# kenoogl/CubeZ

Measured on AMD Instinct MI355X. Metric: MLUPS (lattice updates/s), 512^3 FP32 Jacobi per GPU, higher is better.
Workload: dtype f32

## Files before the change

### cubez_amd/csrc/cz_k_jac3.h

```cpp

template <class T>
__device__ __forceinline__ T* uniform_global(T* p) {
  auto g = (__attribute__((address_space(1))) T*)p;
  asm("" : "+s"(g));
  return (T*)g;
}

__device__ __forceinline__ unsigned lane_offset(unsigned o) {
  asm("" : "+v"(o));
  return o;
}

template <int V>
__device__ __forceinline__ void complete_here(Vec<V>& x) {
  static_assert(V == 2 || V == 4, "one constraint per component");
  if constexpr (V == 4) asm volatile("" : "+v"(x.v[0]), "+v"(x.v[1]), "+v"(x.v[2]), "+v"(x.v[3]));
  else asm volatile("" : "+v"(x.v[0]), "+v"(x.v[1]));
}

template <int V, int TB, int UNIT, int MED, int GATE = 0>
__global__ void __launch_bounds__(TB, 1)
jac3_k(const REAL* __restrict__ U, const REAL* __restrict__ B, REAL* __restrict__ W, Coef c, Geom2 g, double* partials,
       const int* __restrict__ skip, Fin2 fin) {
  if (skip != nullptr && *skip != 0) return;
  extern __shared__ __attribute__((aligned(16))) char smem[];
  const int t = threadIdx.x;
  const int R = g.R;
  constexpr int LV = TB;
  const DeepLds<V> lds = deep_lds<V, LV, 3>(smem, R);
  const int LU = lds.LU;
  Vec<V>* ldsU = lds.U;
  Vec<V>* ldsF = lds.F;
  double* wsum = lds.wsum;

  const PassItem it = pass_item<V>(g);
  const int ja = it.ja, jb = it.jb;

  double acc1 = 0.0, acc2 = 0.0, acc3 = 0.0;
  const typename std::conditional<GATE != 0, GatedDiv<MED>, typename std::conditional<MED != 0, MediumDiv, HoistedDiv>::type>::type dv{fastdiv_init(c.dd)};

  if (it.work) {
    const long long e2_0 = it.fb - 2 * (long long)R;
    const size_t PB = (size_t)g.PSB;
    const RowView<V> rv = row_view<V>(g, it);
    const int x = t;
    const long long f = e2_0 + x;
    unsigned bo = rv.off_of(f);
    const VecMask mk = vec_mask<V>(g, it, f);
    const unsigned inbox = mk.rows ? mk.bits : 0u;
    const unsigned own = (x >= 2 * R && x < LV - 2 * R && mk.rows && mk.kown) ? mk.bits : 0u;
    const bool wave2 = __builtin_amdgcn_ballot_w64(x >= R && x < LV - R) != 0ull;
    const bool wave3 = __builtin_amdgcn_ballot_w64(own != 0) != 0ull;
    OuterRow h = outer_row<V, TB>(rv, LV, it.fb - 3 * (long long)R, f);
    const bool waveh = __builtin_amdgcn_ballot_w64(h.has) != 0ull;
    const char* Ub = reinterpret_cast<const char*>(U);
    const char* Bb = reinterpret_cast<const char*>(B);
    char* Wb = reinterpret_cast<char*>(W);

    const int q0 = ja - 2;
    Vec<V> uA, uB, bA, bB, hx = zerov<V>();
    {
      const Vec<V> t2 = ld16<V>(Ub + (size_t)rv.pl(q0 - 1) * PB, rv.lim(bo, rv.pl(q0 - 1)));
      const Vec<V> t1 = ld16<V>(Ub + (size_t)rv.pl(q0) * PB, rv.lim(bo, rv.pl(q0)));
      Vec<V> h1 = zerov<V>();
      if (waveh) {
        h1 = ld16<V>(Ub + (size_t)rv.pl(q0) * PB, rv.lim(h.bo, rv.pl(q0)));
        hx = ld16<V>(Ub + (size_t)rv.pl(q0 + 1) * PB, rv.lim(h.bo, rv.pl(q0 + 1)));
      }
      uA = ld16<V>(Ub + (size_t)rv.pl(q0 + 1) * PB, rv.lim(bo, rv.pl(q0 + 1)));
      bA = ld16<V>(Bb + (size_t)rv.pl(q0) * PB, rv.lim(bo, rv.pl(q0)));
      ldsU[(size_t)((q0 - 1) & 1) * LU + R + x] = t2;
      ldsU[(size_t)(q0 & 1) * LU + R + x] = t1;
      if (h.has) ldsU[(size_t)(q0 & 1) * LU + h.hl] = h1;
    }
    Vec<V> bq1 = zerov<V>(), bq2 = zerov<V>();
    __syncthreads();

    const int x_first = __builtin_amdgcn_readfirstlane(x), x_last = __builtin_amdgcn_readlane(x, 63);
    auto stage = [&](const Vec<V>* cur, const Vec<V>* prv, const Vec<V>& nxt, const Vec<V>& bb, unsigned msk, unsigned cnt,
                     double& acc) __attribute__((always_inline)) -> Vec<V> {
      const Vec<V> pc = lds_ld<V>(cur + x);
      const Vec<V> im = lds_ld<V>(cur + x - R);
      const Vec<V> ip = lds_ld<V>(cur + x + R);
      const Vec<V> pm = lds_ld<V>(prv + x);
      const REAL elo = reinterpret_cast<const REAL*>(cur)[(long long)x_first * V - 1];
      const REAL ehi = reinterpret_cast<const REAL*>(cur)[(long long)(x_last + 1) * V];
      const REAL kl = lane_shr1(elo, pc.v[V - 1]);
      const REAL kr = lane_shl1(ehi, pc.v[0]);
      return relax_vec<V, UNIT>(pc, im, ip, pm, nxt, kl, kr, bb, c, dv, msk, cnt, acc);
    };

    const char* uN = Ub;
    const char* bN = Bb;
    char* wN = Wb;
    auto step = [&](auto inner, const int q, Vec<V>& uc, Vec<V>& un, Vec<V>& b1, Vec<V>& bn, Vec<V>& b2, Vec<V>& b3) __attribute__((always_inline)) {
      constexpr bool INNER = decltype(inner)::value;
      const char *up, *bp;
      unsigned uo, bo1, ho;
      if constexpr (INNER) {
        uN = uniform_global(uN), bN = uniform_global(bN), wN = uniform_global(wN);
        bo = lane_offset(bo), h.bo = lane_offset(h.bo);
        up = uN, bp = bN, uo = bo, bo1 = bo, ho = h.bo;
      } else {
        const int qu = rv.pl(q + 2 <= jb + 3 ? q + 2 : jb + 3), qb = rv.pl(q + 1 <= jb + 2 ? q + 1 : jb + 2);
        up = Ub + (size_t)qu * PB, bp = Bb + (size_t)qb * PB;
        uo = rv.lim(bo, qu), bo1 = rv.lim(bo, qb), ho = rv.lim(h.bo, qu);
      }
      un = ld16<V>(up, uo);
      bn = ld16<V>(bp, bo1);
      const int p1 = q, p2 = q - 1, p3 = q - 2;
      auto upd = [&](int p) -> unsigned { return (INNER || (p >= g.jj0 && p <= g.jj1)) ? inbox : 0u; };
      auto cnt = [&](int p) -> unsigned { return (INNER || (p >= ja && p <= jb)) ? own : 0u; };
      const Vec<V>* cU = ldsU + (size_t)(p1 & 1) * LU + R;
      const Vec<V>* pU = ldsU + (size_t)((p1 - 1) & 1) * LU + R;
      Vec<V>* F1 = ldsF;
      Vec<V>* F2 = ldsF + (size_t)2 * LV;
      Vec<V> v1 = stage(cU, pU, uc, b1, upd(p1), cnt(p1), acc1);
      complete_here<V>(v1);
      if (waveh) {
        if (h.has) ldsU[(size_t)((p1 + 1) & 1) * LU + h.hl] = hx;
        hx = ld16<V>(up, ho);
      }
      Vec<V> v2 = v1;
      if (wave2) v2 = stage(F1 + (size_t)(p2 & 1) * LV, F1 + (size_t)((p2 - 1) & 1) * LV, v1, b2, upd(p2), cnt(p2), acc2);
      if ((INNER || p3 >= ja) && wave3) {
        const Vec<V> o = stage(F2 + (size_t)(p3 & 1) * LV, F2 + (size_t)((p3 - 1) & 1) * LV, v2, b3, own, own, acc3);
        store_owned<V>(INNER ? wN : Wb + (size_t)p3 * PB, bo, own, o);
      }
      F1[(size_t)(p1 & 1) * LV + x] = v1;
      F2[(size_t)(p2 & 1) * LV + x] = v2;
      Vec<V>* nU = ldsU + (size_t)((p1 + 1) & 1) * LU;
      nU[R + x] = uc;
      if constexpr (!INNER) b3 = b2, b2 = b1;
      if constexpr (INNER) uN += PB, bN += PB, wN += PB;
      __syncthreads();
    };
    const int qi = jb < g.jlast - 3 ? jb : g.jlast - 3;
    int q = q0;
#pragma nounroll
    for (int phase = 0; phase < 2; phase++) {
      const int qg = phase == 0 ? ja + 1 : jb + 2;
      for (;;) {
        step(std::false_type{}, q, uA, uB, bA, bB, bq1, bq2);
        if (++q > qg) break;
        step(std::false_type{}, q, uB, uA, bB, bA, bq1, bq2);
        if (++q > qg) break;
      }
      if (phase == 0) {
        uN = Ub + (size_t)(q + 2) * PB, bN = Bb + (size_t)(q + 1) * PB, wN = Wb + (size_t)(q - 2) * PB;
        for (; q + 3 <= qi; q += 4) {
          step(std::true_type{}, q, uA, uB, bA, bB, bq1, bq2);
          step(std::true_type{}, q + 1, uB, uA, bB, bq2, bA, bq1);
          step(std::true_type{}, q + 2, uA, uB, bq2, bq1, bB, bA);
          step(std::true_type{}, q + 3, uB, uA, bq1, bA, bq2, bB);
        }
      }
    }
  }

  const double acc[3] = {acc1, acc2, acc3};
  pass_epilogue<TB, 3>(acc, partials, fin, wsum);
}
```

### cubez_amd/csrc/cz_k_pass.h

```cpp
struct Geom2 {
  int R;
  long long PSV;
  int nkp = 0;
  long long PSB = 0;
  int jlast = 0;
  unsigned last_off = 0;
  int nwin = 1;
  int hv = 0;
  int KT = 1 << 30;
  int KW = 0;
  int nsegw = 0;
  int kk0, kk1, jj0, jj1;
  long long F0, Fend;
  int kk0a, kk1a, jj0a, jj1a;
  long long F0a, Fenda;
  int nseg, TJ, S;
  int par;
  int zero_u;
  int band;
  const int* map;
};

struct BSrc {
  const REAL* x = nullptr;
  const REAL* y = nullptr;
  const REAL* z = nullptr;
  REAL* out = nullptr;
  REAL a = 0, b = 0;
  const REAL* pa = nullptr;
};

struct Fin2 {
  double* dst = nullptr;
  int do_check = 0, itr = 0;
  int single = 0;
  const double* extra = nullptr;
  int n_extra = 0;
  double res_normal = 0.0, eps = 0.0;
  double* hist = nullptr;
  int* flag = nullptr;
  int* conv_itr = nullptr;
  unsigned* counter = nullptr;
};

template <int V>
__device__ __forceinline__ unsigned colour_bits(int base) {
  const unsigned even = (V == 4) ? 0x5u : (V == 2) ? 0x1u : 0x1u;
  const unsigned odd = (V == 4) ? 0xAu : (V == 2) ? 0x2u : 0x0u;
  return (base & 1) ? odd : even;
}

struct PlainDiv {
  REAL d;
  __device__ __forceinline__ REAL operator()(REAL n) const { return n / d; }
};
struct HoistedDiv {
  FastDiv<REAL> f;
  __device__ __forceinline__ REAL operator()(REAL n) const { return fastdiv(n, f); }
};

struct ShortDiv {
  FastDiv<REAL> f;
  __device__ __forceinline__ REAL operator()(REAL n) const { return shortdiv(n, f); }
};

struct MediumDiv {
  FastDiv<REAL> f;
  __device__ __forceinline__ REAL operator()(REAL n) const { return mediumdiv(n, f); }
};

__device__ __forceinline__ float uniform_real(float x) { return __builtin_bit_cast(float, __builtin_amdgcn_readfirstlane(__builtin_bit_cast(int, x))); }
__device__ __forceinline__ double uniform_real(double x) {
  const unsigned long long b = __builtin_bit_cast(unsigned long long, x);
  const unsigned lo = __builtin_amdgcn_readfirstlane((unsigned)b), hi = __builtin_amdgcn_readfirstlane((unsigned)(b >> 32));
  return __builtin_bit_cast(double, ((unsigned long long)hi << 32) | lo);
}
template <int MED>
struct GatedDiv {
  FastDiv<REAL> f;
  REAL T;
  __device__ __forceinline__ explicit GatedDiv(const FastDiv<REAL>& f_) : f(f_), T(uniform_real(f_.T)) {}
  template <int V>
  __device__ __forceinline__ void vec(const REAL (&n)[V], REAL (&q)[V]) const {
    if (__builtin_expect(gated_none_huge<V>(n, T), 1)) {
#pragma unroll
      for (int cc = 0; cc < V; cc++) q[cc] = gated_tail<MED>(n[cc], f);
    } else {
#pragma unroll
      for (int cc = 0; cc < V; cc++) q[cc] = general_tail<MED>(n[cc], f);
    }
  }
};
template <class DIV>
struct has_vec_entry : std::false_type {};
template <int MED>
struct has_vec_entry<GatedDiv<MED>> : std::true_type {};

template <int V, int UNIT = 0, class DIV>
__device__ __forceinline__ Vec<V> relax_vec(const Vec<V>& pc, const Vec<V>& im, const Vec<V>& ip, const Vec<V>& pm,
                                            const Vec<V>& pn, REAL kl, REAL kr, const Vec<V>& bb, const Coef& c, const DIV& dv,
                                            unsigned mask, unsigned count_mask, double& acc) {
  Vec<V> o;
#if defined(CZ_P2_RES_GROUP)
  REAL grp = (REAL)0;
#endif
  constexpr bool BY_VECTOR = has_vec_entry<DIV>::value;
  REAL nv[V], qv[V];
  if constexpr (BY_VECTOR) {
#pragma unroll
    for (int cc = 0; cc < V; cc++) {
      const REAL km1 = (cc == 0) ? kl : pc.v[cc > 0 ? cc - 1 : 0];
      const REAL kp1 = (cc == V - 1) ? kr : pc.v[cc < V - 1 ? cc + 1 : V - 1];
      nv[cc] = offdiag_sum<UNIT>(c, ip.v[cc], im.v[cc], pn.v[cc], pm.v[cc], kp1, km1) - bb.v[cc];
    }
    dv.template vec<V>(nv, qv);
  }
#pragma unroll
  for (int cc = 0; cc < V; cc++) {
    const REAL pp = pc.v[cc];
    REAL qd;
    if constexpr (BY_VECTOR) {
      qd = qv[cc];
    } else {
      const REAL km1 = (cc == 0) ? kl : pc.v[cc > 0 ? cc - 1 : 0];
      const REAL kp1 = (cc == V - 1) ? kr : pc.v[cc < V - 1 ? cc + 1 : V - 1];
      const REAL ss = offdiag_sum<UNIT>(c, ip.v[cc], im.v[cc], pn.v[cc], pm.v[cc], kp1, km1);
      qd = dv(ss - bb.v[cc]);
    }
    const REAL dp = (qd - pp) * c.omg;
    const REAL d2 = dp * dp;
    o.v[cc] = (mask & (1u << cc)) ? pp + dp : pp;
#if defined(CZ_P2_NO_RES)
    (void)d2, (void)count_mask, (void)acc;
#elif defined(CZ_P2_RES_GROUP)
    grp += (count_mask & (1u << cc)) ? d2 : (REAL)0;
#else
    acc += (double)((count_mask & (1u << cc)) ? d2 : (REAL)0);
#endif
  }
#if defined(CZ_P2_RES_GROUP)
  acc += (double)grp;
#endif
  return o;
}

template <int V>
__device__ __forceinline__ Vec<V> relax_vec_maf(const Vec<V>& pc, const Vec<V>& im, const Vec<V>& ip, const Vec<V>& pm, const Vec<V>& pn,
                                                REAL kl, REAL kr, const Vec<V>& bb, REAL XG, REAL XGG, REAL YE, REAL YEE, const Vec<V>& ZT,
                                                const Vec<V>& ZTT, REAL omg, unsigned mask, unsigned count_mask, double& acc) {
  Vec<V> o;
#pragma unroll
  for (int cc = 0; cc < V; cc++) {
    const REAL pp = pc.v[cc];
    const REAL km1 = (cc == 0) ? kl : pc.v[cc > 0 ? cc - 1 : 0];
    const REAL kp1 = (cc == V - 1) ? kr : pc.v[cc < V - 1 ? cc + 1 : V - 1];
    const MafW w = maf_weights(XG, XGG, YE, YEE, ZT.v[cc], ZTT.v[cc]);
    const REAL rp = w.w1 * ip.v[cc] + w.w2 * im.v[cc] + w.w3 * pn.v[cc] + w.w4 * pm.v[cc] + w.w5 * kp1 + w.w6 * km1 + bb.v[cc];
    const REAL dp = (rp / w.dd - pp) * omg;
    const REAL d2 = dp * dp;
    o.v[cc] = (mask & (1u << cc)) ? pp + dp : pp;
    acc += (double)((count_mask & (1u << cc)) ? d2 : (REAL)0);
  }
  return o;
}

template <int V>
__device__ __forceinline__ Vec<V> ld16(const char* plane, unsigned byte_off) {
  typedef typename NatVec<V>::type nv;
  typedef nv unv __attribute__((aligned(sizeof(REAL))));
  const nv x = *reinterpret_cast<const unv*>(plane + byte_off);
  Vec<V> r;
  __builtin_memcpy(&r, &x, sizeof(r));
  return r;
}
template <int V>
__device__ __forceinline__ void st16(char* plane, unsigned byte_off, const Vec<V>& x) {
  typedef typename NatVec<V>::type nv;
  typedef nv unv __attribute__((aligned(sizeof(REAL))));
  nv y;
  __builtin_memcpy(&y, &x, sizeof(y));
  *reinterpret_cast<unv*>(plane + byte_off) = y;
}

template <int V>
__device__ __forceinline__ Vec<V> lds_ld(const Vec<V>* p) {
  typedef typename NatVec<V>::type nv;
  nv x = *reinterpret_cast<const nv*>(p);
  asm("" : "+v"(x));
  Vec<V> r;
  __builtin_memcpy(&r, &x, sizeof(r));
  return r;
}

struct PassItem {
  int win, seg, chunk;
  int kw0;
  long long fb;
  int ja, jb;
  bool work;
};
template <int V>
__device__ __forceinline__ PassItem pass_item(const Geom2& g) {
  PassItem it;
  const int lb = blockIdx.x;
  int seg, chunk;
  if (g.map != nullptr) {
    seg = g.map[2 * lb];
    chunk = g.map[2 * lb + 1];
  } else {
    const int x = lb & 7, r = lb >> 3;
    const int base = g.nseg >> 3, rem = g.nseg & 7, bmax = base + (rem ? 1 : 0);
    const int blen = base + (x < rem ? 1 : 0);
    const int sl = r % bmax;
    chunk = r / bmax;
    seg = (sl < blen) ? x * base + min(x, rem) + sl : g.nseg;
  }
  int win = 0;
  if (g.nwin > 1 && seg < g.nseg) {
    win = seg / g.nsegw;
    seg -= win * g.nsegw;
  } else if (g.nwin > 1) {
    seg = g.nsegw;
  }
  const int nseg_w = (g.nwin > 1) ? g.nsegw : g.nseg;
  it.win = win, it.seg = seg, it.chunk = chunk;
  it.kw0 = win * g.KW - g.hv * V;
  it.fb = (seg < nseg_w) ? g.F0 + (long long)seg * g.S : g.Fend;
  it.ja = g.jj0 + chunk * g.TJ;
  it.jb = it.ja + g.TJ - 1;
  if (it.jb > g.jj1) it.jb = g.jj1;
  it.work = it.ja <= it.jb && it.fb < g.Fend;
  return it;
}

template <int V>
struct RowView {
  int R, nkp, kw0, jlast;
  unsigned last_off;
  long long vlast;
  __device__ __forceinline__ unsigned off_of(long long f) const {
    if (f < 0) f = 0;
    if (f > vlast) f = vlast;
    const long long r = f / R;
    long long el = r * nkp + kw0 + (f - r * R) * V;
    el = el < 0 ? 0 : el;
    return (unsigned)(el * (long long)sizeof(REAL));
  }
  __device__ __forceinline__ unsigned lim(unsigned off, int plane) const { return plane == jlast ? (off < last_off ? off : last_off) : off; }
  __device__ __forceinline__ int pl(int p) const { return p < 0 ? 0 : (p > jlast ? jlast : p); }
};
template <int V>
__device__ __forceinline__ RowView<V> row_view(const Geom2& g, const PassItem& it) {
  return RowView<V>{g.R, g.nkp, it.kw0, g.jlast, g.last_off, g.PSV - 1};
}

struct VecMask {
  unsigned bits, bits1;
  bool rows, rows1;
  bool kown;
  int pbase;
};
template <int V>
__device__ __forceinline__ VecMask vec_mask(const Geom2& g, const PassItem& it, long long f) {
  const long long fc = f < 0 ? 0 : f;
  const long long row = fc / g.R;
  const int kv = (int)(fc - row * g.R);
  const int kb = it.kw0 + kv * V;
  VecMask m;
  m.bits = 0, m.bits1 = 0;
#pragma unroll
  for (int cc = 0; cc < V; cc++) {
    const int kk = kb + cc;
    if (kk >= g.kk0a && kk <= g.kk1a) m.bits1 |= 1u << cc;
    if (kk >= g.kk0 && kk <= g.kk1) m.bits |= 1u << cc;
  }
  m.rows = f >= g.F0 && f < g.Fend;
  m.rows1 = f >= g.F0a && f < g.Fenda;
  m.kown = kv >= g.hv && kv < g.hv + g.KT;
  m.pbase = kb + (int)row + g.par;
  return m;
}

struct OuterRow {
  bool has;
  int hl;
  unsigned bo;
};
template <int V, int TB>
__device__ __forceinline__ OuterRow outer_row(const RowView<V>& rv, int LV, long long f_outer0, long long f_own) {
  const int t = threadIdx.x, R = rv.R;
  OuterRow h;
  h.has = (t < R) || (t >= TB - R);
  h.hl = (t < R) ? t : (LV + R + (t - (TB - R)));
  h.bo = rv.off_of(h.has ? f_outer0 + h.hl : f_own);
  return h;
}

template <int V>
__device__ __forceinline__ void store_owned(char* plane, unsigned bo, unsigned own, const Vec<V>& x) {
  if (own == (1u << V) - 1) {
    st16<V>(plane, bo, x);
  } else if (own != 0) {
    REAL* p = reinterpret_cast<REAL*>(plane + bo);
#pragma unroll
    for (int cc = 0; cc < V; cc++)
      if (own & (1u << cc)) p[cc] = x.v[cc];
  }
}

template <int V>
struct DeepLds {
  int LU;
  Vec<V>* U;
  Vec<V>* F;
  double* wsum;
};
template <int V, int LV, int D>
__device__ __forceinline__ DeepLds<V> deep_lds(char* smem, int R) {
  DeepLds<V> l;
  l.LU = LV + 2 * R;
  l.U = reinterpret_cast<Vec<V>*>(smem) + R;
  l.F = l.U + (size_t)2 * l.LU;
  l.wsum = reinterpret_cast<double*>(l.F + (size_t)(2 * (D - 1)) * LV + R);
  return l;
}

template <int TB, int N>
__device__ __forceinline__ void pass_finalize(const double* partials, int nblk, const Fin2& fin, double* wsum) {
  const int t = threadIdx.x;
  double x[N];
#pragma unroll
  for (int s = 0; s < N; s++) x[s] = 0.0;
  for (int i = t; i < nblk; i += TB) {
#pragma unroll
    for (int s = 0; s < N; s++) x[s] += __hip_atomic_load(&partials[s * nblk + i], __ATOMIC_RELAXED, __HIP_MEMORY_SCOPE_AGENT);
  }
  for (int i = t; i < fin.n_extra; i += TB) {
#pragma unroll
    for (int s = 0; s < N; s++) x[s] += fin.extra[s * fin.n_extra + i];
  }
  double tot[N];
#pragma unroll
  for (int s = 0; s < N; s++) {
    __syncthreads();
    tot[s] = block_sum<TB>(x[s], wsum);
  }
  if (t == 0) {
    const bool single = N == 2 && fin.single;
    if (single) tot[0] = tot[0] + tot[1];
    const int nit = single ? 1 : N;
    for (int s = 0; s < nit; s++) fin.dst[s] = tot[s];
    if (fin.do_check) {
      for (int s = 0; s < nit; s++) {
        const double r = sqrt(tot[s] * fin.res_normal);
        fin.hist[fin.itr + s] = r;
        if (r < fin.eps) {
          *fin.flag = 1;
          *fin.conv_itr = fin.itr + s;
          break;
        }
      }
    }
    *fin.counter = 0u;
  }
}

template <int TB, int N>
__device__ __forceinline__ void pass_epilogue(const double (&acc)[N], double* partials, const Fin2& fin, double* wsum) {
  const int lb = blockIdx.x, nblk = gridDim.x;
  double s[N];
#pragma unroll
  for (int n = 0; n < N; n++) {
    __syncthreads();
    s[n] = block_sum<TB>(acc[n], wsum);
  }
  int* last_flag = reinterpret_cast<int*>(wsum + 16);
  if (threadIdx.x == 0) {
#pragma unroll
    for (int n = 0; n < N; n++) __hip_atomic_store(&partials[n * nblk + lb], s[n], __ATOMIC_RELAXED, __HIP_MEMORY_SCOPE_AGENT);
    *last_flag = arrive_and_test_last(fin.counter, nblk);
  }
  __syncthreads();
  if (*last_flag) pass_finalize<TB, N>(partials, nblk, fin, wsum);
}
```

### cubez_amd/csrc/cz_k_rb4.h

```cpp
template <int V, int TB, int UNIT>
__global__ void __launch_bounds__(TB, 1)
rb4_k(const REAL* __restrict__ U, const REAL* __restrict__ B, REAL* __restrict__ W, Coef c, Geom2 g, double* partials,
      const int* __restrict__ skip, Fin2 fin) {
  if (skip != nullptr && *skip != 0) return;
  extern __shared__ __attribute__((aligned(16))) char smem[];
  const int t = threadIdx.x;
  const int R = g.R;
  constexpr int LV = TB;
  const DeepLds<V> lds = deep_lds<V, LV, 4>(smem, R);
  const int LU = lds.LU;
  Vec<V>* ldsU = lds.U;
  Vec<V>* ldsF = lds.F;
  double* wsum = lds.wsum;

  const PassItem it = pass_item<V>(g);
  const int ja = it.ja, jb = it.jb;

  double acc1 = 0.0, acc2 = 0.0;
  const HoistedDiv dv{fastdiv_init(c.dd)};

  if (it.work) {
    const long long e3_0 = it.fb - 3 * (long long)R;
    const size_t PB = (size_t)g.PSB;
    const RowView<V> rv = row_view<V>(g, it);
    int x;
    {
      const int off = (int)(((e3_0 % R) + R) % R);
      const int L0 = off == 0 ? R : R - off;
      int nA = L0;
      for (int st = L0 + R; st < LV; st += 2 * R) nA += min(R, LV - st);
      if (t < nA) {
        const int m = t - L0, j = m / R;
        x = t < L0 ? t : L0 + R + 2 * R * j + (m - j * R);
      } else {
        const int n = t - nA, j = n / R;
        x = L0 + 2 * R * j + (n - j * R);
      }
    }
    const long long f = e3_0 + x;
    const unsigned bo = rv.off_of(f);
    const VecMask mk = vec_mask<V>(g, it, f);
    const int pbase = mk.pbase;
    const unsigned inbox = mk.rows ? mk.bits : 0u;
    const unsigned own = (x >= 3 * R && x < LV - 3 * R && mk.rows && mk.kown) ? mk.bits : 0u;
    const OuterRow h = outer_row<V, TB>(rv, LV, it.fb - 4 * (long long)R, f);
    const char* Ub = reinterpret_cast<const char*>(U);
    const char* Bb = reinterpret_cast<const char*>(B);
    char* Wb = reinterpret_cast<char*>(W);

    const int q0 = ja - 3;
    Vec<V> uA, uB, bA, bB, hx;
    {
      const Vec<V> t2 = ld16<V>(Ub + (size_t)rv.pl(q0 - 1) * PB, rv.lim(bo, rv.pl(q0 - 1)));
      const Vec<V> t1 = ld16<V>(Ub + (size_t)rv.pl(q0) * PB, rv.lim(bo, rv.pl(q0)));
      const Vec<V> h1 = ld16<V>(Ub + (size_t)rv.pl(q0) * PB, rv.lim(h.bo, rv.pl(q0)));
      uA = ld16<V>(Ub + (size_t)rv.pl(q0 + 1) * PB, rv.lim(bo, rv.pl(q0 + 1)));
      bA = ld16<V>(Bb + (size_t)rv.pl(q0) * PB, rv.lim(bo, rv.pl(q0)));
      ldsU[(size_t)((q0 - 1) & 1) * LU + R + x] = t2;
      ldsU[(size_t)(q0 & 1) * LU + R + x] = t1;
      if (h.has) ldsU[(size_t)(q0 & 1) * LU + h.hl] = h1;
    }
    Vec<V> bq1 = zerov<V>(), bq2 = zerov<V>(), bq3 = zerov<V>();
    __syncthreads();

    const int x_first = __builtin_amdgcn_readfirstlane(x), x_last = __builtin_amdgcn_readlane(x, 63);
    struct Ops {
      Vec<V> pc, im, ip;
      REAL elo, ehi;
    };
    auto fetch = [&](const Vec<V>* cur) __attribute__((always_inline)) -> Ops {
      Ops o;
      o.pc = lds_ld<V>(cur + x);
      o.im = lds_ld<V>(cur + x - R);
      o.ip = lds_ld<V>(cur + x + R);
      o.elo = reinterpret_cast<const REAL*>(cur)[(long long)x_first * V - 1];
      o.ehi = reinterpret_cast<const REAL*>(cur)[(long long)(x_last + 1) * V];
      return o;
    };
    auto compute = [&](const Ops& o, const Vec<V>* cur, const Vec<V>* prv, const Vec<V>& nxt, const Vec<V>& bb, int p, int colour, unsigned msk, unsigned cnt, double& acc,
                       const bool first = false) __attribute__((always_inline)) -> Vec<V> {
      const Vec<V> pm = lds_ld<V>(prv + x);
      const REAL kl = lane_shr1(o.elo, o.pc.v[V - 1]);
      REAL kr = lane_shl1(o.ehi, o.pc.v[0]);
      if (first) kr = (x == LV - 1) ? reinterpret_cast<const REAL*>(cur)[(long long)LV * V] : kr;
      const bool sc = ((pbase + p + colour) & 1) != 0;
      return relax_vec_rb_branch<V>(o.pc, o.im, o.ip, pm, nxt, kl, kr, bb, sc, msk, cnt, acc,
                             [&](REAL pp, REAL ipv, REAL imv, REAL pnv, REAL pmv, REAL kp1, REAL km1, REAL bv, REAL, REAL) {
                               const REAL ss = offdiag_sum<UNIT>(c, ipv, imv, pnv, pmv, kp1, km1);
                               return (dv(ss - bv) - pp) * c.omg;
                             });
    };

    auto step = [&](const int q, Vec<V>& uc, Vec<V>& un, Vec<V>& b1, Vec<V>& bn) __attribute__((always_inline)) {
      {
        const int qu = rv.pl(q + 2 <= jb + 4 ? q + 2 : jb + 4), qb = rv.pl(q + 1 <= jb + 3 ? q + 1 : jb + 3);
        hx = ld16<V>(Ub + (size_t)rv.pl(q + 1) * PB, rv.lim(h.bo, rv.pl(q + 1)));
        un = ld16<V>(Ub + (size_t)qu * PB, rv.lim(bo, qu));
        bn = ld16<V>(Bb + (size_t)qb * PB, rv.lim(bo, qb));
      }
      const int p1 = q, p2 = q - 1, p3 = q - 2, p4 = q - 3;
      auto upd = [&](int p) -> unsigned { return (p >= g.jj0 && p <= g.jj1) ? inbox : 0u; };
      auto cnt = [&](int p) -> unsigned { return (p >= ja && p <= jb) ? own : 0u; };
      const Vec<V>* cU = ldsU + (size_t)(p1 & 1) * LU + R;
      const Vec<V>* pU = ldsU + (size_t)((p1 - 1) & 1) * LU + R;
      Vec<V>* F1 = ldsF;
      Vec<V>* F2 = ldsF + (size_t)2 * LV;
      Vec<V>* F3 = ldsF + (size_t)4 * LV;
      const Ops o1 = fetch(cU);
      const Ops o2 = fetch(F1 + (size_t)(p2 & 1) * LV);
      const Vec<V> v1 = compute(o1, cU, pU, uc, b1, p1, 0, upd(p1), cnt(p1), acc1, true);
      const Ops o3 = fetch(F2 + (size_t)(p3 & 1) * LV);
      const Vec<V> v2 = compute(o2, nullptr, F1 + (size_t)((p2 - 1) & 1) * LV, v1, bq1, p2, 1, upd(p2), cnt(p2), acc1);
      const Ops o4 = fetch(F3 + (size_t)(p4 & 1) * LV);
      const Vec<V> v3 = compute(o3, nullptr, F2 + (size_t)((p3 - 1) & 1) * LV, v2, bq2, p3, 0, upd(p3), cnt(p3), acc2);
      if (p4 >= ja && __builtin_amdgcn_ballot_w64(own != 0) != 0ull) {
        const Vec<V> o = compute(o4, nullptr, F3 + (size_t)((p4 - 1) & 1) * LV, v3, bq3, p4, 1, own, own, acc2);
        store_owned<V>(Wb + (size_t)p4 * PB, bo, own, o);
      }
      F1[(size_t)(p1 & 1) * LV + x] = v1;
      F2[(size_t)(p2 & 1) * LV + x] = v2;
      F3[(size_t)(p3 & 1) * LV + x] = v3;
      Vec<V>* nU = ldsU + (size_t)((p1 + 1) & 1) * LU;
      nU[R + x] = uc;
      if (h.has) nU[h.hl] = hx;
      bq3 = bq2, bq2 = bq1, bq1 = b1;
      __syncthreads();
    };
    for (int q = q0;; q += 2) {
      step(q, uA, uB, bA, bB);
      if (q + 1 > jb + 3) break;
      step(q + 1, uB, uA, bB, bA);
      if (q + 2 > jb + 3) break;
    }
  }

  const double acc[2] = {acc1, acc2};
  pass_epilogue<TB, 2>(acc, partials, fin, wsum);
}
```

Measured before the change: 1.080 million.

## Port jac3 inner-loop specialization to rb4 kernel with rotating B registers

Moves the uniform_global, lane_offset and complete_here helpers into the shared pass header so the red-black 4-stage kernel can use them. The rb4 step is split into boundary and inner variants: the inner loop walks scalar base pointers with no clamping or range checks and is unrolled by six, rotating the B pipeline registers instead of copying them. Halo loads are skipped for waves with no halo lanes and issued mid-step to overlap with compute, and wave-uniform ballots gate the owned stage. The aim is less address arithmetic, fewer register moves and fewer scalar/vector conversions per plane, at the cost of more code and higher register pressure.

```diff
diff --git a/cubez_amd/csrc/cz_k_jac3.h b/cubez_amd/csrc/cz_k_jac3.h
--- a/cubez_amd/csrc/cz_k_jac3.h
+++ b/cubez_amd/csrc/cz_k_jac3.h
@@ -1,22 +1,4 @@
 
-template <class T>
-__device__ __forceinline__ T* uniform_global(T* p) {
-  auto g = (__attribute__((address_space(1))) T*)p;
-  asm("" : "+s"(g));
-  return (T*)g;
-}
-
-__device__ __forceinline__ unsigned lane_offset(unsigned o) {
-  asm("" : "+v"(o));
-  return o;
-}
-
-template <int V>
-__device__ __forceinline__ void complete_here(Vec<V>& x) {
-  static_assert(V == 2 || V == 4, "one constraint per component");
-  if constexpr (V == 4) asm volatile("" : "+v"(x.v[0]), "+v"(x.v[1]), "+v"(x.v[2]), "+v"(x.v[3]));
-  else asm volatile("" : "+v"(x.v[0]), "+v"(x.v[1]));
-}
 
 template <int V, int TB, int UNIT, int MED, int GATE = 0>
 __global__ void __launch_bounds__(TB, 1)
diff --git a/cubez_amd/csrc/cz_k_pass.h b/cubez_amd/csrc/cz_k_pass.h
--- a/cubez_amd/csrc/cz_k_pass.h
+++ b/cubez_amd/csrc/cz_k_pass.h
@@ -192,6 +192,25 @@
   return r;
 }
 
+template <class T>
+__device__ __forceinline__ T* uniform_global(T* p) {
+  auto g = (__attribute__((address_space(1))) T*)p;
+  asm("" : "+s"(g));
+  return (T*)g;
+}
+
+__device__ __forceinline__ unsigned lane_offset(unsigned o) {
+  asm("" : "+v"(o));
+  return o;
+}
+
+template <int V>
+__device__ __forceinline__ void complete_here(Vec<V>& x) {
+  static_assert(V == 2 || V == 4, "one constraint per component");
+  if constexpr (V == 4) asm volatile("" : "+v"(x.v[0]), "+v"(x.v[1]), "+v"(x.v[2]), "+v"(x.v[3]));
+  else asm volatile("" : "+v"(x.v[0]), "+v"(x.v[1]));
+}
+
 struct PassItem {
   int win, seg, chunk;
   int kw0;
diff --git a/cubez_amd/csrc/cz_k_rb4.h b/cubez_amd/csrc/cz_k_rb4.h
--- a/cubez_amd/csrc/cz_k_rb4.h
+++ b/cubez_amd/csrc/cz_k_rb4.h
@@ -38,22 +38,28 @@
       }
     }
     const long long f = e3_0 + x;
-    const unsigned bo = rv.off_of(f);
+    unsigned bo = rv.off_of(f);
     const VecMask mk = vec_mask<V>(g, it, f);
     const int pbase = mk.pbase;
     const unsigned inbox = mk.rows ? mk.bits : 0u;
     const unsigned own = (x >= 3 * R && x < LV - 3 * R && mk.rows && mk.kown) ? mk.bits : 0u;
-    const OuterRow h = outer_row<V, TB>(rv, LV, it.fb - 4 * (long long)R, f);
+    const bool wave4 = __builtin_amdgcn_ballot_w64(own != 0) != 0ull;
+    OuterRow h = outer_row<V, TB>(rv, LV, it.fb - 4 * (long long)R, f);
+    const bool waveh = __builtin_amdgcn_ballot_w64(h.has) != 0ull;
     const char* Ub = reinterpret_cast<const char*>(U);
     const char* Bb = reinterpret_cast<const char*>(B);
     char* Wb = reinterpret_cast<char*>(W);
 
     const int q0 = ja - 3;
-    Vec<V> uA, uB, bA, bB, hx;
+    Vec<V> uA, uB, bA, bB, hx = zerov<V>();
     {
       const Vec<V> t2 = ld16<V>(Ub + (size_t)rv.pl(q0 - 1) * PB, rv.lim(bo, rv.pl(q0 - 1)));
       const Vec<V> t1 = ld16<V>(Ub + (size_t)rv.pl(q0) * PB, rv.lim(bo, rv.pl(q0)));
-      const Vec<V> h1 = ld16<V>(Ub + (size_t)rv.pl(q0) * PB, rv.lim(h.bo, rv.pl(q0)));
+      Vec<V> h1 = zerov<V>();
+      if (waveh) {
+        h1 = ld16<V>(Ub + (size_t)rv.pl(q0) * PB, rv.lim(h.bo, rv.pl(q0)));
+        hx = ld16<V>(Ub + (size_t)rv.pl(q0 + 1) * PB, rv.lim(h.bo, rv.pl(q0 + 1)));
+      }
       uA = ld16<V>(Ub + (size_t)rv.pl(q0 + 1) * PB, rv.lim(bo, rv.pl(q0 + 1)));
       bA = ld16<V>(Bb + (size_t)rv.pl(q0) * PB, rv.lim(bo, rv.pl(q0)));
       ldsU[(size_t)((q0 - 1) & 1) * LU + R + x] = t2;
@@ -61,6 +67,7 @@
       if (h.has) ldsU[(size_t)(q0 & 1) * LU + h.hl] = h1;
     }
     Vec<V> bq1 = zerov<V>(), bq2 = zerov<V>(), bq3 = zerov<V>();
+    Vec<V> bX = zerov<V>();
     __syncthreads();
 
     const int x_first = __builtin_amdgcn_readfirstlane(x), x_last = __builtin_amdgcn_readlane(x, 63);
@@ -84,23 +91,36 @@
       REAL kr = lane_shl1(o.ehi, o.pc.v[0]);
       if (first) kr = (x == LV - 1) ? reinterpret_cast<const REAL*>(cur)[(long long)LV * V] : kr;
       const bool sc = ((pbase + p + colour) & 1) != 0;
-      return relax_vec_rb_branch<V>(o.pc, o.im, o.ip, pm, nxt, kl, kr, bb, sc, msk, cnt, acc,
+      const Vec<V> r = relax_vec_rb_branch<V>(o.pc, o.im, o.ip, pm, nxt, kl, kr, bb, sc, msk, cnt, acc,
                              [&](REAL pp, REAL ipv, REAL imv, REAL pnv, REAL pmv, REAL kp1, REAL km1, REAL bv, REAL, REAL) {
                                const REAL ss = offdiag_sum<UNIT>(c, ipv, imv, pnv, pmv, kp1, km1);
                                return (dv(ss - bv) - pp) * c.omg;
                              });
+      asm volatile("" : "+v"(acc));
+      return r;
     };
 
-    auto step = [&](const int q, Vec<V>& uc, Vec<V>& un, Vec<V>& b1, Vec<V>& bn) __attribute__((always_inline)) {
-      {
+    const char* uN = Ub;
+    const char* bN = Bb;
+    char* wN = Wb;
+    auto step = [&](auto inner, const int q, Vec<V>& uc, Vec<V>& un, Vec<V>& b1, Vec<V>& bn, Vec<V>& b2, Vec<V>& b3, Vec<V>& b4) __attribute__((always_inline)) {
+      constexpr bool INNER = decltype(inner)::value;
+      const char *up, *bp;
+      unsigned uo, bo1, ho;
+      bo = lane_offset(bo), h.bo = lane_offset(h.bo);
+      if constexpr (INNER) {
+        uN = uniform_global(uN), bN = uniform_global(bN), wN = uniform_global(wN);
+        up = uN, bp = bN, uo = bo, bo1 = bo, ho = h.bo;
+      } else {
         const int qu = rv.pl(q + 2 <= jb + 4 ? q + 2 : jb + 4), qb = rv.pl(q + 1 <= jb + 3 ? q + 1 : jb + 3);
-        hx = ld16<V>(Ub + (size_t)rv.pl(q + 1) * PB, rv.lim(h.bo, rv.pl(q + 1)));
-        un = ld16<V>(Ub + (size_t)qu * PB, rv.lim(bo, qu));
-        bn = ld16<V>(Bb + (size_t)qb * PB, rv.lim(bo, qb));
+        up = uniform_global(Ub + (size_t)qu * PB), bp = uniform_global(Bb + (size_t)qb * PB);
+        uo = rv.lim(bo, qu), bo1 = rv.lim(bo, qb), ho = rv.lim(h.bo, qu);
       }
+      un = ld16<V>(up, uo);
+      bn = ld16<V>(bp, bo1);
       const int p1 = q, p2 = q - 1, p3 = q - 2, p4 = q - 3;
-      auto upd = [&](int p) -> unsigned { return (p >= g.jj0 && p <= g.jj1) ? inbox : 0u; };
-      auto cnt = [&](int p) -> unsigned { return (p >= ja && p <= jb) ? own : 0u; };
+      auto upd = [&](int p) -> unsigned { return (INNER || (p >= g.jj0 && p <= g.jj1)) ? inbox : 0u; };
+      auto cnt = [&](int p) -> unsigned { return (INNER || (p >= ja && p <= jb)) ? own : 0u; };
       const Vec<V>* cU = ldsU + (size_t)(p1 & 1) * LU + R;
       const Vec<V>* pU = ldsU + (size_t)((p1 - 1) & 1) * LU + R;
       Vec<V>* F1 = ldsF;
@@ -108,29 +128,52 @@
       Vec<V>* F3 = ldsF + (size_t)4 * LV;
       const Ops o1 = fetch(cU);
       const Ops o2 = fetch(F1 + (size_t)(p2 & 1) * LV);
-      const Vec<V> v1 = compute(o1, cU, pU, uc, b1, p1, 0, upd(p1), cnt(p1), acc1, true);
+      Vec<V> v1 = compute(o1, cU, pU, uc, b1, p1, 0, upd(p1), cnt(p1), acc1, true);
+      complete_here<V>(v1);
+      complete_here<V>(uc), complete_here<V>(b1);
+      if (waveh) {
+        if (h.has) ldsU[(size_t)((p1 + 1) & 1) * LU + (int)lane_offset((unsigned)h.hl)] = hx;
+        hx = ld16<V>(up, ho);
+      }
       const Ops o3 = fetch(F2 + (size_t)(p3 & 1) * LV);
-      const Vec<V> v2 = compute(o2, nullptr, F1 + (size_t)((p2 - 1) & 1) * LV, v1, bq1, p2, 1, upd(p2), cnt(p2), acc1);
+      const Vec<V> v2 = compute(o2, nullptr, F1 + (size_t)((p2 - 1) & 1) * LV, v1, b2, p2, 1, upd(p2), cnt(p2), acc1);
       const Ops o4 = fetch(F3 + (size_t)(p4 & 1) * LV);
-      const Vec<V> v3 = compute(o3, nullptr, F2 + (size_t)((p3 - 1) & 1) * LV, v2, bq2, p3, 0, upd(p3), cnt(p3), acc2);
-      if (p4 >= ja && __builtin_amdgcn_ballot_w64(own != 0) != 0ull) {
-        const Vec<V> o = compute(o4, nullptr, F3 + (size_t)((p4 - 1) & 1) * LV, v3, bq3, p4, 1, own, own, acc2);
-        store_owned<V>(Wb + (size_t)p4 * PB, bo, own, o);
+      const Vec<V> v3 = compute(o3, nullptr, F2 + (size_t)((p3 - 1) & 1) * LV, v2, b3, p3, 0, upd(p3), cnt(p3), acc2);
+      if ((INNER || p4 >= ja) && wave4) {
+        const Vec<V> o = compute(o4, nullptr, F3 + (size_t)((p4 - 1) & 1) * LV, v3, b4, p4, 1, own, own, acc2);
+        store_owned<V>(INNER ? wN : Wb + (size_t)p4 * PB, bo, own, o);
       }
       F1[(size_t)(p1 & 1) * LV + x] = v1;
       F2[(size_t)(p2 & 1) * LV + x] = v2;
       F3[(size_t)(p3 & 1) * LV + x] = v3;
       Vec<V>* nU = ldsU + (size_t)((p1 + 1) & 1) * LU;
       nU[R + x] = uc;
-      if (h.has) nU[h.hl] = hx;
-      bq3 = bq2, bq2 = bq1, bq1 = b1;
+      if constexpr (!INNER) b4 = b3, b3 = b2, b2 = b1;
+      if constexpr (INNER) uN += PB, bN += PB, wN += PB;
       __syncthreads();
     };
-    for (int q = q0;; q += 2) {
-      step(q, uA, uB, bA, bB);
-      if (q + 1 > jb + 3) break;
-      step(q + 1, uB, uA, bB, bA);
-      if (q + 2 > jb + 3) break;
+    const int qi = jb < g.jlast - 3 ? jb : g.jlast - 3;
+    int q = q0;
+#pragma nounroll
+    for (int phase = 0; phase < 2; phase++) {
+      const int qg = phase == 0 ? ja + 2 : jb + 3;
+      for (;;) {
+        step(std::false_type{}, q, uA, uB, bA, bB, bq1, bq2, bq3);
+        if (++q > qg) break;
+        step(std::false_type{}, q, uB, uA, bB, bA, bq1, bq2, bq3);
+        if (++q > qg) break;
+      }
+      if (phase == 0) {
+        uN = Ub + (size_t)(q + 2) * PB, bN = Bb + (size_t)(q + 1) * PB, wN = Wb + (size_t)(q - 3) * PB;
+        for (; q + 5 <= qi; q += 6) {
+          step(std::true_type{}, q, uA, uB, bA, bB, bq1, bq2, bq3);
+          step(std::true_type{}, q + 1, uB, uA, bB, bX, bA, bq1, bq2);
+          step(std::true_type{}, q + 2, uA, uB, bX, bq3, bB, bA, bq1);
+          step(std::true_type{}, q + 3, uB, uA, bq3, bq2, bX, bB, bA);
+          step(std::true_type{}, q + 4, uA, uB, bq2, bq1, bq3, bX, bB);
+          step(std::true_type{}, q + 5, uB, uA, bq1, bA, bq2, bq3, bX);
+        }
+      }
     }
   }
 
```

Result: no change. 1.079 million (-0.1%).
